# marja-w/gan-des-midi-music-gen

Measured on AMD Instinct MI355X. Metric: GAN training samples/sec (G+D step), higher is better.
Workload: dtype bf16; 1 GPU; SIMNN G/D iteration, synthetic 128x256 spectrogram windows; per_gpu_batch=256, global_batch=256, mode=faithful, parallelism=dp1

## Files before the change

gan_des_midi_music_gen_amd/_lib.py:

```python
import ctypes
import os
import threading

_PKG = os.path.dirname(os.path.abspath(__file__))
_TAG = os.environ.get("GDM_LIB_TAG", "")
LIB_PATH = os.path.join(_PKG, "libgdm_hip" + (f"_{_TAG}" if _TAG else "") + ".so")

F32, BF16 = 0, 1
ACT_NONE, ACT_RELU, ACT_LEAKY, ACT_SIGMOID = 0, 1, 2, 3
CRITERIA = {"bce": 0, "mse": 1, "l1": 2}
PCM_U8, PCM_S16, PCM_S24, PCM_S32, PCM_F32 = range(5)
PCM_BYTES = (1, 2, 3, 4, 4)

_c = ctypes
_P, _I, _L, _F, _Z = _c.c_void_p, _c.c_int, _c.c_int64, _c.c_float, _c.c_size_t

class LinearBnJob(_c.Structure):
    _fields_ = [(n, _P) for n in ("x", "w", "bias", "gamma", "beta", "running_mean", "running_var",
                                  "num_batches_tracked", "y_out", "out", "save_mean", "save_invstd")] + \
               [(n, _I) for n in ("M", "N", "K", "groups", "stat_repeats")]


class DcnnAdam(_c.Structure):
    _fields_ = [("param", _P * 6), ("exp_avg", _P * 6), ("exp_avg_sq", _P * 6), ("hyper", _P), ("done", _P)]


class ConcatJob(_c.Structure):
    _fields_ = [("a", _P), ("b", _P), ("out", _P), ("M", _I), ("Ka", _I), ("Kb", _I)]


SIGNATURES = {
    "gdm_last_error": (_c.c_char_p, []),
    "gdm_version": (_I, []),
    "gdm_arch": (_c.c_char_p, []),
    "gdm_build_flavor": (_I, []),
    "gdm_gemm": (_I, [_P, _I, _L, _L, _P, _I, _L, _L, _P, _I, _L, _L, _I, _I, _I, _P, _P, _I, _F, _I, _I, _P, _Z, _P]),
    "gdm_gemm_plan": (_I, [_P, _I, _L, _L, _P, _I, _L, _L, _P, _I, _L, _L, _I, _I, _I, _P, _I, _I, _P]),
    "gdm_bce_with_logits": (_I, [_P, _F, _I, _F, _P, _P, _I, _I, _P]),
    "gdm_criterion_loss": (_I, [_P, _F, _I, _I, _F, _P, _P, _I, _P]),
    "gdm_adam_step": (_I, [_P, _P, _P, _P, _L, _I, _F, _F, _F, _F, _F, _P]),
    "gdm_adam_step_dev": (_I, [_P, _P, _P, _P, _L, _P, _P]),
    "gdm_adam_step_dev_pc": (_I, [_P, _P, _P, _P, _I, _I, _I, _P, _I, _P, _I, _P]),
    "gdm_stft_frames": (_I, [_P, _I, _L, _L, _I, _I, _I, _P, _P]),
    "gdm_power_spectrum": (_I, [_P, _L, _I, _I, _P, _P]),
    "gdm_power_to_db": (_I, [_P, _I, _I, _I, _F, _F, _P, _P]),
    "gdm_pcm_to_float": (_I, [_P, _I, _I, _I, _L, _L, _L, _P, _P]),
    "gdm_pcm_stft_frames": (_I, [_P, _I, _I, _I, _L, _L, _L, _I, _L, _L, _I, _I, _I, _P, _P]),
    "gdm_bn_workspace_bytes": (_Z, [_I, _I]),
    "gdm_bn_act_fwd": (_I, [_P, _I, _I, _P, _P, _P, _P, _P, _F, _F, _I, _P, _I, _P, _P, _I, _P, _Z, _P]),
    "gdm_bn_act_bwd": (_I, [_P, _P, _I, _P, _I, _I, _P, _P, _P, _I, _P, _P, _P, _P, _Z, _P]),
    "gdm_bn_stats": (_I, [_P, _I, _I, _P, _P, _P, _F, _F, _P, _P, _P, _Z, _P]),
    "gdm_bn_partial_chunks": (_I, [_I]),
    "gdm_bn_partials": (_I, [_P, _I, _I, _P, _P]),
    "gdm_bn_apply": (_I, [_P, _I, _I, _P, _P, _P, _P, _I, _P, _I, _P]),
    "gdm_bn_finalize": (_I, [_P, _I, _I, _I, _F, _F, _P, _P, _P, _P, _P, _P]),
    "gdm_simnn_gen_pack_bytes": (_Z, []),
    "gdm_simnn_gen_pack": (_I, [_P, _I, _P, _P, _P, _P]),
    "gdm_simnn_gen_first": (_I, [_P, _I, _I, _P, _P, _F, _F, _P, _P, _P, _P, _P, _P]),
    "gdm_simnn_gen_convt_chunks": (_I, [_I, _I]),
    "gdm_simnn_gen_convt_bn": (_I, [_I, _P, _P, _P, _P, _P, _I, _P, _P, _P, _P]),
    "gdm_simnn_gen_last": (_I, [_P, _P, _P, _P, _P, _P, _I, _P, _P]),
    "gdm_simnn_gen_eval": (_I, [_P, _I, _I, _P, _P] + [_P] * 12 + [_F, _P, _P, _P, _P, _P, _P]),
    "gdm_bias_act_fwd": (_I, [_P, _P, _I, _I, _I, _F, _P, _I, _P]),
    "gdm_act_bwd": (_I, [_P, _P, _I, _L, _I, _F, _P, _P]),
    "gdm_colsum": (_I, [_P, _I, _I, _I, _P, _P, _Z, _P]),
    "gdm_cast": (_I, [_P, _I, _P, _I, _L, _P]),
    "gdm_nonfinite_count": (_I, [_P, _I, _L, _P, _P]),
    "gdm_simnn_conv1_fwd": (_I, [_P, _P, _P, _I, _I, _I, _P, _P, _I, _P]),
    "gdm_simnn_conv1_fwd_pair": (_I, [_P, _P, _I, _P, _P, _I, _I, _I, _P, _P, _I, _P]),
    "gdm_simnn_conv2_pack_bytes": (_Z, [_I]),
    "gdm_simnn_conv2_pack": (_I, [_P, _I, _P, _P]),
    "gdm_simnn_conv2_fwd": (_I, [_P, _P, _P, _I, _I, _I, _P, _P, _I, _P]),
    "gdm_simnn_conv2_bwd_fused_workspace_bytes": (_Z, [_I, _I, _I]),
    "gdm_simnn_conv2_bwd_fused": (_I, [_P, _P, _P, _I, _I, _I, _P, _P, _P, _I, _I, _I, _P, _I, _P, _Z, _P]),
    "gdm_simnn_conv2_bwd_fused_finish": (_I, [_I, _I, _I, _P, _P, _P, _Z, _P]),
    "gdm_simnn_conv2_bwd_data": (_I, [_P, _P, _P, _I, _I, _I, _P, _I, _P]),
    "gdm_simnn_conv2_bwd_weight_workspace_bytes": (_Z, [_I, _I, _I]),
    "gdm_simnn_conv2_bwd_weight": (_I, [_P, _P, _P, _I, _I, _I, _P, _P, _I, _P, _Z, _P]),
    "gdm_simnn_conv1_bwd_weight_workspace_bytes": (_Z, [_I, _I, _I]),
    "gdm_simnn_conv1_bwd_weight": (_I, [_P, _P, _P, _I, _I, _I, _P, _P, _I, _I, _P, _Z, _P]),
    "gdm_simnn_conv1_bwd_data": (_I, [_P, _P, _P, _I, _I, _I, _P, _I, _P]),
    "gdm_simnn_adam_step": (_I, [_P, _P, _P, _P, _I, _I, _I, _P, _P, _P, _P, _P, _I, _P, _P, _I, _P, _P, _P]),
    "gdm_simnn_head_workspace_bytes": (_Z, [_I]),
    "gdm_simnn_head": (_I, [_P, _P, _P, _I, _I, _F, _F, _P, _P, _I, _P, _I, _P, _P, _P, _P, _Z, _P]),
    "gdm_linear_bn_act_max_rows": (_I, []),
    "gdm_linear_bn_act_fwd_multi": (_I, [_P, _I, _F, _F, _I, _I, _P]),
    "gdm_concat_cols_multi": (_I, [_P, _I, _P]),
    "gdm_linear_bn_act_fwd": (_I, [_P, _P, _P, _P, _P, _P, _P, _P, _F, _F, _I, _I, _I, _I, _I, _P, _P, _P, _P, _I, _I,
                                   _P]),
    "gdm_dcnn_fused_supported": (_I, [_I]),
    "gdm_dcnn_pack_bytes": (_Z, [_I]),
    "gdm_dcnn_pack": (_I, [_P, _P, _P, _P, _P, _P, _I, _P, _P]),
    "gdm_dcnn_fused_workspace_bytes": (_Z, [_I, _I, _I]),
    "gdm_dcnn_fused": (_I, [_P, _I, _P, _P, _I, _I, _F, _F, _P, _P, _P, _I, _I, _P, _P, _P, _P, _P, _P, _P, _Z, _P]),
    "gdm_dcnn_fused_adam": (_I, [_P, _I, _P, _P, _I, _I, _F, _F, _P, _P, _P, _I, _P, _P, _P, _P, _P, _P, _P, _P, _Z, _P]),
    "gdm_dcnn_fused_crit": (_I, [_P, _I, _P, _P, _I, _I, _F, _F, _P, _P, _P, _I, _I, _P, _P, _P, _P, _P, _P, _I, _P, _Z,
                                 _P]),
    "gdm_dcnn_fused_adam_crit": (_I, [_P, _I, _P, _P, _I, _I, _F, _F, _P, _P, _P, _I, _P, _P, _P, _P, _P, _P, _P, _I, _P,
                                      _Z, _P]),
    "gdm_im2col": (_I, [_P, _I, _I, _I, _I, _I, _I, _I, _I, _I, _I, _I, _I, _P, _I, _P]),
    "gdm_col2im": (_I, [_P, _I, _I, _I, _I, _I, _I, _I, _I, _I, _I, _I, _P, _I, _I, _P]),
    "gdm_permute_pc": (_I, [_P, _I, _I, _I, _I, _P, _I, _P]),
    "gdm_des_scan": (_I, [_P, _L, _I, _I, _I, _F, _I, _I, _P, _P, _P, _P, _P, _P, _P]),
    "gdm_des_routing": (_I, [_P, _L, _I, _I, _I, _P, _P, _P, _P]),
    "gdm_des_run": (_I, [_P, _I, _P, _P, _P, _L, _L, _L, _P, _P, _P, _P, _P, _L, _P, _P]),
    "gdm_piano_roll_raster": (_I, [_P, _P, _P, _I, _I, _P, _P, _P]),
    "gdm_piano_roll_windows": (_I, [_P, _P, _P, _P, _P, _I, _I, _P, _P, _P]),
    "gdm_des_log_to_roll": (_I, [_P, _P, _P, _P, _P, _L, _P, _I, _P, _P, _I, _P, _I, _I, _I, _I, _P, _I, _P, _I, _P, _P,
                                 _P]),
    "gdm_maxpool2_fwd": (_I, [_P, _I, _I, _I, _I, _I, _P, _P, _P]),
    "gdm_maxpool2_bwd": (_I, [_P, _I, _P, _I, _I, _I, _I, _P, _P]),
}

_lock = threading.Lock()
_lib = None


class GdmError(RuntimeError):
    pass


def load():
    global _lib
    if _lib is not None:
        return _lib
    with _lock:
        if _lib is None:
            if not os.path.exists(LIB_PATH):
                raise GdmError(
                    f"{LIB_PATH} is missing: build it with `python -m gan_des_midi_music_gen_amd.build` "
                    "(hipcc --offload-arch=gfx950). There is no CPU or eager-PyTorch fallback for this path.")
            import torch
            lib = ctypes.CDLL(LIB_PATH)
            for name, (res, args) in SIGNATURES.items():
                fn = getattr(lib, name)
                fn.restype, fn.argtypes = res, args
            _lib = lib
    return _lib


def check(rc, what):
    if rc != 0:
        msg = load().gdm_last_error().decode(errors="replace")
        raise GdmError(f"{what} failed (rc={rc}): {msg}")
```

gan_des_midi_music_gen_amd/ops.py:

```python
import contextlib
import ctypes
import threading

import torch

from . import _lib
from ._lib import ACT_LEAKY, ACT_NONE, ACT_RELU, ACT_SIGMOID, BF16, CRITERIA, F32, GdmError, check
from ._lib import PCM_BYTES, PCM_F32, PCM_S16, PCM_S24, PCM_S32, PCM_U8

_TORCH_DT = {F32: torch.float32, BF16: torch.bfloat16}


def torch_dtype(dt):
    return _TORCH_DT[dt]


def gdm_dtype(t):
    if t.dtype == torch.float32:
        return F32
    if t.dtype == torch.bfloat16:
        return BF16
    raise GdmError(f"unsupported tensor dtype {t.dtype} (fp32 or bf16 only)")


# ... 486 lines not shown
        assert dw.numel() == 64 and db.numel() == 16 and dw.is_contiguous() and db.is_contiguous()
    else:
        dw = torch.empty((16, 1, 2, 2), dtype=torch.float32, device=x0.device)
        db = torch.empty(16, dtype=torch.float32, device=x0.device)
    dp1 = torch.empty((b, h1, w1, 16), dtype=dp2.dtype, device=dp2.device) if want_dp1 else None
    lib = _lib.load()
    nb = lib.gdm_simnn_conv2_bwd_fused_workspace_bytes(b, h1, w1)
    ws = workspace(nb, x0.device)
    _call("gdm_simnn_conv2_bwd_fused", _p(dp2), _p(code2), _p(pack), b, h1, w1, _p(code1), _p(x0), _p(x1), bsplit, h,
          wd, _p(dp1), gdm_dtype(dp2), _p(ws), nb, _stream())
    _call("gdm_simnn_conv2_bwd_fused_finish", b, h1, w1, _p(dw), _p(db), _p(ws), nb, _stream())
    return dw, db, dp1


def simnn_conv2_bwd_weight(dp2, code2, p1, out=None):
    _need_gpu(dp2, code2, p1)
    assert dp2.is_contiguous() and code2.is_contiguous() and p1.is_contiguous() and dp2.dtype == p1.dtype
    b, h1, w1, _ = p1.shape
    if out is not None:
        dw, db = out
        assert dw.numel() == 4608 and db.numel() == 32 and dw.is_contiguous() and db.is_contiguous()
    else:
        dw = torch.empty((32, 16, 3, 3), dtype=torch.float32, device=p1.device)
        db = torch.empty(32, dtype=torch.float32, device=p1.device)
    lib = _lib.load()
    nb = lib.gdm_simnn_conv2_bwd_weight_workspace_bytes(b, h1, w1)
    ws = workspace(nb, p1.device)
    _call("gdm_simnn_conv2_bwd_weight", _p(dp2), _p(code2), _p(p1), b, h1, w1, _p(dw), _p(db), gdm_dtype(p1), _p(ws),
                                         nb, _stream())
    return dw, db


def simnn_conv1_bwd_weight(dp1, code1, x, out=None, accumulate=False):
    _need_gpu(dp1, code1, x)
    assert dp1.is_contiguous() and code1.is_contiguous() and x.is_contiguous()
    b, h, wd = x.shape
    assert dp1.shape[0] == b and code1.shape == (b, (h + 1) // 2, simnn_code1_width((wd + 1) // 2))
    if out is not None:
        dw, db = out
        assert dw.numel() == 64 and db.numel() == 16 and dw.is_contiguous() and db.is_contiguous()
    else:
        assert not accumulate
        dw = torch.empty((16, 1, 2, 2), dtype=torch.float32, device=x.device)
        db = torch.empty(16, dtype=torch.float32, device=x.device)
    lib = _lib.load()
    nb = lib.gdm_simnn_conv1_bwd_weight_workspace_bytes(b, h, wd)
    ws = workspace(nb, x.device)
    _call("gdm_simnn_conv1_bwd_weight", _p(dp1), _p(code1), _p(x), b, h, wd, _p(dw), _p(db), gdm_dtype(dp1),
                                         1 if accumulate else 0, _p(ws), nb, _stream())
    return dw, db


def simnn_conv1_bwd_data(dp1, code1, w, h, wd):
    _need_gpu(dp1, code1, w)
    assert dp1.is_contiguous() and code1.is_contiguous() and w.is_contiguous() and w.numel() == 64
    b = dp1.shape[0]
    assert dp1.shape == (b, (h + 1) // 2, (wd + 1) // 2, 16)
    assert code1.shape == (b, (h + 1) // 2, simnn_code1_width((wd + 1) // 2))
    dx = torch.empty((b, h, wd), dtype=torch.float32, device=dp1.device)
    _call("gdm_simnn_conv1_bwd_data", _p(dp1), _p(code1), _p(w), b, h, wd, _p(dx), gdm_dtype(dp1), _stream())
    return dx


def simnn_head(h1, w2, b2, n0, y0, y1, *, loss_out, accumulate_loss=False, want_grad=True, grad_out=None, dh_dtype=F32):
    _need_gpu(h1, w2, b2, loss_out)
    assert h1.dim() == 2 and h1.shape[1] == 128 and h1.is_contiguous() and h1.dtype == torch.float32
    n = h1.shape[0]
    prob = torch.empty(n, dtype=torch.float32, device=h1.device)
    dh1 = dw2 = db2 = db1 = None
    if want_grad:
        dh1 = torch.empty(h1.shape, dtype=_TORCH_DT[dh_dtype], device=h1.device)
        if grad_out is not None:
            dw2, db2, db1 = grad_out
            assert dw2.numel() == 128 and db2.numel() == 1 and db1.numel() == 128
        else:
            dw2 = torch.empty((1, 128), dtype=torch.float32, device=h1.device)
            db2 = torch.empty(1, dtype=torch.float32, device=h1.device)
            db1 = torch.empty(128, dtype=torch.float32, device=h1.device)
    nb = _lib.load().gdm_simnn_head_workspace_bytes(n)
    ws = workspace(nb, h1.device)
    _call("gdm_simnn_head", _p(h1), _p(w2), _p(b2), n, n0, float(y0), float(y1), _p(prob), _p(loss_out),
          1 if accumulate_loss else 0, _p(dh1), int(dh_dtype), _p(dw2), _p(db2), _p(db1), _p(ws), nb, _stream())
    return prob, dh1, ((dw2, db2, db1) if want_grad else None)


def linear_bn_act_max_rows():
    return _lib.load().gdm_linear_bn_act_max_rows()


def linear_bn_act_fwd(x, w, bias, gamma, beta, running_mean, running_var, nbt, *, act, training=True, momentum=0.1,
                      eps=1e-5, save_y=False, groups=1, stat_repeats=1):
    _need_gpu(x, w, bias, gamma, beta, running_mean, running_var, nbt)
    assert x.dim() == 2 and w.dim() == 2 and x.shape[1] == w.shape[1] and x.is_contiguous() and w.is_contiguous()
    assert x.dtype == torch.float32 and w.dtype == torch.float32
    rows, k = x.shape
    assert rows % groups == 0
    m = rows // groups
    n = w.shape[0]
    out = torch.empty((rows, n), dtype=torch.float32, device=x.device)
    y = torch.empty((rows, n), dtype=torch.float32, device=x.device) if save_y else None
    shape = (n,) if groups == 1 else (groups, n)
    mean = torch.empty(shape, dtype=torch.float32, device=x.device)
    invstd = torch.empty(shape, dtype=torch.float32, device=x.device)
    _call("gdm_linear_bn_act_fwd", _p(x), _p(w), _p(bias), _p(gamma), _p(beta), _p(running_mean), _p(running_var),
          _p(nbt), float(momentum), float(eps), act, 1 if training else 0, m, n, k, _p(y), _p(out), _p(mean),
          _p(invstd), int(groups), int(stat_repeats), _stream())
    return out, y, mean, invstd


def linear_bn_act_fwd_multi(jobs, *, act, training=True, momentum=0.1, eps=1e-5):
    assert 1 <= len(jobs) <= 2
    arr = (_lib.LinearBnJob * len(jobs))()
    res = []
    for i, j in enumerate(jobs):
        x, w = j["x"], j["w"]
        _need_gpu(x, w, j["bias"], j["gamma"], j["beta"], j["running_mean"], j["running_var"], j["nbt"])
        assert x.dim() == 2 and w.dim() == 2 and x.shape[1] == w.shape[1] and x.is_contiguous() and w.is_contiguous()
        assert x.dtype == torch.float32 and w.dtype == torch.float32
        groups, reps = int(j.get("groups", 1)), int(j.get("stat_repeats", 1))
        rows, k = x.shape
        assert rows % groups == 0
        n = w.shape[0]
        out = torch.empty((rows, n), dtype=torch.float32, device=x.device)
        shape = (n,) if groups == 1 else (groups, n)
        mean = torch.empty(shape, dtype=torch.float32, device=x.device)
        invstd = torch.empty(shape, dtype=torch.float32, device=x.device)
        a = arr[i]
        a.x, a.w, a.bias, a.gamma, a.beta = _p(x), _p(w), _p(j["bias"]), _p(j["gamma"]), _p(j["beta"])
        a.running_mean, a.running_var, a.num_batches_tracked = _p(j["running_mean"]), _p(j["running_var"]), _p(j["nbt"])
        a.y_out, a.out, a.save_mean, a.save_invstd = None, _p(out), _p(mean), _p(invstd)
        a.M, a.N, a.K, a.groups, a.stat_repeats = rows // groups, n, k, groups, reps
        res.append((out, mean, invstd))
    _call("gdm_linear_bn_act_fwd_multi", ctypes.cast(arr, ctypes.c_void_p), len(jobs), float(momentum), float(eps), act,
          1 if training else 0, _stream())
    return res


def concat_cols_multi(pairs, outs=None):
    assert 1 <= len(pairs) <= 4 and (outs is None or len(outs) == len(pairs))
    arr = (_lib.ConcatJob * len(pairs))()
    res = []
    for i, (a, b) in enumerate(pairs):
        _need_gpu(a, b)
        assert a.dim() == 2 and b.dim() == 2 and a.shape[0] == b.shape[0] and a.is_contiguous() and b.is_contiguous()
        assert a.dtype == torch.float32 and b.dtype == torch.float32
        shape = (a.shape[0], a.shape[1] + b.shape[1])
        out = outs[i] if outs is not None else torch.empty(shape, dtype=torch.float32, device=a.device)
        assert tuple(out.shape) == shape and out.is_contiguous() and out.dtype == torch.float32
        q = arr[i]
        q.a, q.b, q.out, q.M, q.Ka, q.Kb = _p(a), _p(b), _p(out), a.shape[0], a.shape[1], b.shape[1]
        res.append(out)
    _call("gdm_concat_cols_multi", ctypes.cast(arr, ctypes.c_void_p), len(pairs), _stream())
    return res


def dcnn_fused_supported(t):
    return bool(_lib.load().gdm_dcnn_fused_supported(int(t)))


def dcnn_pack(w1, b1, w2, b2, wfc, bfc, t, out=None):
    _need_gpu(w1, b1, w2, b2, wfc, bfc, out)
    for a in (w1, b1, w2, b2, wfc, bfc):
        assert a.dtype == torch.float32 and a.is_contiguous()
    nbytes = _lib.load().gdm_dcnn_pack_bytes(int(t))
    pack = out if out is not None else torch.empty(nbytes, dtype=torch.uint8, device=w1.device)
    assert pack.numel() == nbytes
# ... 317 lines not shown
```

gan_des_midi_music_gen_amd/train.py:

```python
import torch

from . import dp
from . import functional as Fn
from . import ops


class FlatBuffers:

    ALIGN = 64

    def __init__(self, params, extra=0, local=0):
        params = [p for p in params]
        assert params, "no parameters"
        dev = params[0].device
        self.params = params
        self.numel = sum(p.numel() for p in params)
        big = max(range(len(params)), key=lambda i: params[i].numel())
        order = [i for i in range(len(params)) if i != big] + [big]
        n_small = self.numel - params[big].numel()
        assert extra % 4 == 0 and 0 <= local <= extra
        self.n_small = (n_small + self.ALIGN - 1) // self.ALIGN * self.ALIGN
        self.n_pad = self.n_small - n_small
        self.n_extra = extra
        self.n_local = local
# ... 128 lines not shown
            torch.cuda.current_stream().wait_event(self._gen_event)

    def _reduce_big_async(self):
        self._pending = dp.allreduce_async_(self.d.bucket_big(), self.pg)

    def _reduce(self):
        pending = self._pending
        if pending is None:
            red = self.d.bucket_reduced()
            dp.allreduce_bucket_(red, red.numel(), self.pg)
        else:
            dp.allreduce_bucket_(self.d.bucket_head(), self.d.bucket_head().numel(), self.pg)
            pending.wait()
            self._pending = None

    def _adam(self):
        self.d.adam(self.lr, self.betas, self.eps, grad_scale=1.0 / self.world)

    def _reduce_and_step(self):
        self._reduce()
        self._adam()

    def _sync_hyper(self):
        self.d.sync_hyper(self.lr, self.betas, self.eps, 1.0 / self.world)

    @torch.no_grad()
    def load_discriminator_state(self, params=None, exp_avg=None, exp_avg_sq=None, step=None):
        d = self.d
        for src, flat in ((params, d.flat), (exp_avg, d.exp_avg), (exp_avg_sq, d.exp_avg_sq)):
            if src is None:
                continue
            assert len(src) == len(d.views)
            for v, s_ in zip(d.views, src):
                off = (v.data_ptr() - d.flat.data_ptr()) // 4
                flat[off:off + v.numel()].copy_(s_.detach().reshape(-1).to(flat.device, torch.float32))
        if step is not None:
            d.step_count = int(step)
            if d._hyper is not None:
                d._hyper.view(torch.int32)[0:1].copy_(torch.tensor([int(step)], dtype=torch.int32))
                if d.derived_record is not None:
                    d.derived_record.zero_()
        if params is not None:
            self._refresh_operands()

    def _count_nonfinite(self, tensors):
        if self._nf is None:
            self._nf = torch.zeros(1, dtype=torch.int32, device=self.d.flat.device)
        ops.nonfinite_count(tensors, self._nf)
        return self._nf

    def _watch(self, *tensors):
        if torch.is_anomaly_enabled():
            self._count_nonfinite([t for t in tensors if isinstance(t, torch.Tensor)])

    def check_finite(self, *tensors):
        nf = self._count_nonfinite([self.loss_g, self.loss_d, self.d.flat, self.d.exp_avg, self.d.exp_avg_sq, *tensors])
        n = int(nf.item())
        nf.zero_()
        if n:
            raise ops.NonFiniteError(f"{type(self).__name__}: {n} non-finite value(s) in inputs, losses, discriminator "
                                     f"parameters or optimizer state after iteration {self.iterations}")

    def _anomaly_check(self):
        if torch.is_anomaly_enabled() and not torch.cuda.is_current_stream_capturing():
            self.check_finite()

    def disc_loss_value(self):
        return self.loss_d.item() / self.world

    def gen_loss_value(self):
        return self.loss_g.item()

    def gen_loss_global(self):
        if self.world == 1:
            return self.loss_g.item()
        t = self.loss_g.clone()
        dp.allreduce_bucket_(t, 1, self.pg)
        return t.item() / self.world


class SimnnTrainer(_TrainerBase):

    def __init__(self, gen, disc, lr=0.00002, betas=(0.5, 0.999), eps=1e-8, compute_dtype=None,
                 elide_dead_backward=False, process_group=None, overlap=True, one_launch_optimizer=True):
        self.gen, self.disc = gen, disc
        self.one_launch_optimizer = one_launch_optimizer
        self._init_common([disc.conv1.weight, disc.conv1.bias, disc.conv2.weight, disc.conv2.bias, disc.fc1.weight,
                           disc.fc1.bias, disc.fc2.weight, disc.fc2.bias], lr, betas, eps, compute_dtype,
                          elide_dead_backward, process_group)
        self._last_generated = None
        self._prepared = None
        self.overlap = overlap
        self._tm_cache = {}
        self._side = None
        self._pending_fake = None
        self._fake_buf = None
        self._pieces = None
        self._piece_streams = None

    @property
    def last_generated(self):
        self._join_generators()
        return self._last_generated

    def invalidate_weights(self):
        self._prepared = None

    def _refresh_operands(self):
        if self._prepared is not None:
            Fn.simnn_disc_prepare(self.d.views[2], self.d.views[4], self.dt, out=self._prepared)

    def _operands(self):
        if self._prepared is None:
            self._prepared = Fn.simnn_disc_prepare(self.d.views[2], self.d.views[4], self.dt)
        return self._prepared

    def _adam(self):
        wf1 = self.d.views[4]
        n, k = wf1.shape
        d = self.d
        if not self.one_launch_optimizer:
            d.adam(self.lr, self.betas, self.eps, grad_scale=1.0 / self.world, big_pc=(n, 32, k // 32, self._prepared[1]))
            ops.simnn_conv2_pack(d.views[2], self.dt, out=self._prepared[0])
            return
        if self._adam_done is None:
            self._adam_done = d.derived_record = torch.zeros(ops.SIMNN_ADAM_RECORD_INTS, dtype=torch.int32,
                                                             device=d.flat.device)
        hyper = d.hyper_record(self.lr, self.betas, self.eps, 1.0 / self.world)
        ns = d.n_small
        ops.simnn_adam_step(d.flat[ns:], d.grad[ns:], d.exp_avg[ns:], d.exp_avg_sq[ns:], n, 32, k // 32, self._prepared[1],
                            d.flat[:ns], d.grad[:ns], d.exp_avg[:ns], d.exp_avg_sq[:ns], d.views[2], self._prepared[0],
                            hyper, self._adam_done)

    def _gen_state(self):
        g = self.gen
        ws = [g.conv1.weight.detach(), g.conv2.weight.detach(), g.conv3.weight.detach(), g.conv4.weight.detach()]
        bns = [(bn.weight.detach(), bn.bias.detach(), bn.running_mean, bn.running_var, bn.num_batches_tracked)
               for bn in (g.batch_norm1, g.batch_norm2, g.batch_norm3)]
        return ws, bns

    def _streams(self, dev, fork=True):
        if not (self.overlap and fork):
            return None
        if self._side is None:
            self._side = [torch.cuda.Stream(dev) for _ in range(3)]
        return self._side

    def _gen_forward(self, noise, keep):
        ws, bns = self._gen_state()
        self._last_generated, gsaved = Fn.simnn_gen_forward(noise, ws, bns, self.gen.training, self.dt,
                                                            cache=self._tm_cache, need_backward=False)
        keep.append(gsaved)
        return self._last_generated

    def _conv1_pair(self, real, fake):
        w1, b1 = self.d.views[:2]
        b, h, w = real.shape
        h1, w1s = (h + 1) // 2, (w + 1) // 2
        p1 = torch.empty((2 * b, h1, w1s, 16), dtype=ops.torch_dtype(self.dt), device=real.device)
        code1 = torch.empty((2 * b, h1, ops.simnn_code1_width(w1s)), dtype=torch.int64, device=real.device)
        ops.simnn_conv1_fwd(real, w1, b1, self.dt, out=(p1[:b], code1[:b]))
        ops.simnn_conv1_fwd(fake, w1, b1, self.dt, out=(p1[b:], code1[b:]))
        return p1, code1

    def _features_head(self, x, trunk, n0, y0, y1, loss_out, grad_out=None, want_grad=True):
        w1, b1, _w2, b2, _wf1, bf1, wf2, bf2 = self.d.views
        pack, wf1p = self._operands()
        hid, saved = Fn.simnn_disc_features(x, w1, b1, pack, b2, wf1p, bf1, self.dt, trunk_out=trunk)
        prob, dh, _ = ops.simnn_head(hid, wf2, bf2, n0, y0, y1, loss_out=loss_out, want_grad=want_grad,
                                     grad_out=grad_out, dh_dtype=self.dt)
        return saved, dh, (hid, prob)

    def _disc_features_head(self, trunk):
        gv = self.d.grad_views
        return self._features_head(None, trunk, trunk[0].shape[0] // 2, 0.9, 0.1, self.loss_d,
                                   grad_out=(gv[6], gv[7], gv[5]))

    def _fc1_dw(self, saved, dh, outs):
        n, k = self._prepared[1].shape
        ops.gemm(dh.t(), saved[3], compute=self.dt, out=outs[4].view(n, k))

    def _backward_rest(self, saved, dh, outs, x_pair, keep):
        _x, p1, code1, _flat, code2 = saved[:5]
        pack, wf1p = self._prepared
        dflat = ops.gemm(dh, wf1p, compute=self.dt, out_dtype=self.dt)
        dp2 = dflat.view(p1.shape[0], p1.shape[1] // 2, p1.shape[2] // 2, 32)
        keep.append(dflat)
        ops.simnn_conv2_bwd_weight(dp2, code2, p1, out=(outs[2], outs[3]))
        ops.simnn_conv2_bwd_fused(dp2, code2, pack, code1, x_pair[0], x_pair[1], out=(outs[0], outs[1]))

    def _d_backward(self, saved, dh, outs, x_pair, keep, fork=True):
        main = torch.cuda.current_stream()
        side = self._streams(saved[1].device, fork)
        if side:
            side[1].wait_stream(main)
        with torch.cuda.stream(side[1] if side else main):
            self._fc1_dw(saved, dh, outs)
            if self.world > 1 and outs is self.d.grad_views:
                self._reduce_big_async()
        self._backward_rest(saved, dh, outs, x_pair, keep)
        if side:
            main.wait_stream(side[1])

    def _generator_half(self, fake, keep, fork=False):
        saved, dh, head = self._features_head(fake, None, fake.shape[0], 1.0, 1.0, self.loss_g,
                                              want_grad=not self.elide)
        if not self.elide:
            self._d_backward(saved, dh, self._scratch(), (fake, None), keep, fork=fork)
        keep.append((saved, dh, head))

    def _gen_forward_beside(self, noise, keep, side):
        main = torch.cuda.current_stream()
        if side:
            side[0].wait_stream(main)
        with torch.cuda.stream(side[0] if side else main):
            return self._gen_forward(noise, keep)

    @torch.no_grad()
    def step(self, real, noise, fake):
        if self._pending_fake is not None:
            self.flush()
        real = Fn._f32c(real)
        self._watch(real, noise, fake)
        main = torch.cuda.current_stream()
        side = self._streams(real.device)
        keep = []
        bridge = callable(fake)
        if bridge:
            generated = self._gen_forward_beside(noise, keep, side)
            if side:
                main.wait_stream(side[0])
            fake = fake(generated)
        fake = Fn._f32c(fake.to(real.device))
        assert fake.shape == real.shape, (fake.shape, real.shape)
        self._operands()
        trunk = self._conv1_pair(real, fake)
        if not bridge:
            self._gen_forward_beside(noise, keep, side)
        saved, dh, head = self._disc_features_head(trunk)
        self._d_backward(saved, dh, self.d.grad_views, (real, fake), keep)
        self._reduce_and_step()
        self._generator_half(fake, keep, fork=True)
        if side:
            main.wait_stream(side[0])
        self.iterations += 1
        del keep, saved, dh, head
        self._anomaly_check()
        return self.loss_d, self.loss_g

    @torch.no_grad()
    def step_pipelined(self, real, noise, fake, with_generator=True):
        if callable(fake):
            raise ops.GdmError("step_pipelined needs a tensor for the fake batch (the bridge is host code)")
        real = Fn._f32c(real)
        fake = Fn._f32c(fake.to(real.device))
        assert fake.shape == real.shape, (fake.shape, real.shape)
        main = torch.cuda.current_stream()
        side = self._streams(real.device)
        keep = []
        pending = self._pending_fake
        self._operands()
        self._scratch()
        trunk = self._conv1_pair(real, fake)
        if with_generator:
            self._gen_forward_beside(noise, keep, side)
        if side:
            side[2].wait_stream(main)
        with torch.cuda.stream(side[2] if side else main):
# ... 415 lines not shown
```

include/gdm.h:

```cpp
#ifndef GDM_H
#define GDM_H
#include <stddef.h>
#include <stdint.h>

#ifdef __cplusplus
extern "C" {
#endif

enum { GDM_F32 = 0, GDM_BF16 = 1 };
enum { GDM_ACT_NONE = 0, GDM_ACT_RELU = 1, GDM_ACT_LEAKY = 2, GDM_ACT_SIGMOID = 3 };
enum { GDM_OK = 0, GDM_EINVAL = -1, GDM_ELAUNCH = -2, GDM_EWORKSPACE = -3 };
enum { GDM_CRIT_BCE_LOGITS = 0, GDM_CRIT_MSE = 1, GDM_CRIT_L1 = 2 };

const char* gdm_last_error(void);
int gdm_version(void);
const char* gdm_arch(void);
int gdm_build_flavor(void);

int gdm_gemm(const void* A, int a_dtype, int64_t sam, int64_t sak,
             const void* B, int b_dtype, int64_t sbk, int64_t sbn,
             void* C, int c_dtype, int64_t scm, int64_t scn,
             int M, int N, int K,
             const float* bias_n, const float* bias_m, int act, float slope,
             int compute_dtype, int split_k, void* workspace, size_t workspace_bytes, void* stream);
// ... 21 lines not shown
int gdm_adam_step_dev_pc(float* p, const float* g_pc, float* m, float* v, int N, int C, int P, void* shadow_pc,
                         int shadow_dtype, float* hyper, int advance_step, void* stream);

size_t gdm_bn_workspace_bytes(int rows, int channels);
int gdm_bn_act_fwd(const float* y, int rows, int channels, const float* gamma, const float* beta,
                   float* running_mean, float* running_var, int64_t* num_batches_tracked, float momentum, float eps,
                   int act, void* out, int out_dtype, float* save_mean, float* save_invstd, int training,
                   void* workspace, size_t workspace_bytes, void* stream);
int gdm_bn_act_bwd(const void* dout, const void* out, int out_dtype, const float* y, int rows, int channels,
                   const float* gamma, const float* save_mean, const float* save_invstd, int act, float* dy,
                   float* dgamma, float* dbeta, void* workspace, size_t workspace_bytes, void* stream);
int gdm_bn_stats(const float* y, int rows, int channels, float* running_mean, float* running_var,
                 int64_t* num_batches_tracked, float momentum, float eps, float* save_mean, float* save_invstd,
                 void* workspace, size_t workspace_bytes, void* stream);
int gdm_bn_partial_chunks(int rows);
int gdm_bn_partials(const float* y, int rows, int channels, float* partials, void* stream);
int gdm_bn_apply(const float* y, int rows, int channels, const float* gamma, const float* beta, const float* mean,
                 const float* invstd, int act, void* out, int out_dtype, void* stream);
int gdm_bn_finalize(const float* ws, int chunks, int rows, int channels, float momentum, float eps, float* running_mean,
                    float* running_var, int64_t* num_batches_tracked, float* save_mean, float* save_invstd, void* stream);

size_t gdm_simnn_gen_pack_bytes(void);
int gdm_simnn_gen_pack(const float* w1, int noise_dim, const float* w2, const float* w3, void* pack, void* stream);
int gdm_simnn_gen_first(const float* noise, int B, int noise_dim, const void* pack, float* y1, float momentum, float eps,
                        float* running_mean, float* running_var, int64_t* num_batches_tracked, float* save_mean,
                        float* save_invstd, void* stream);
int gdm_simnn_gen_convt_chunks(int layer, int B);
int gdm_simnn_gen_convt_bn(int layer, const float* yin, const float* mean, const float* invstd, const float* gamma,
                           const float* beta, int B, const void* pack, float* yout, float* ws_partials, void* stream);
int gdm_simnn_gen_last(const float* yin, const float* mean, const float* invstd, const float* gamma, const float* beta,
                       const float* w4, int B, float* out, void* stream);
int gdm_simnn_gen_eval(const float* noise, int B, int noise_dim, const void* pack, const float* w4,
                       const float* gamma1, const float* beta1, const float* rmean1, const float* rvar1,
                       const float* gamma2, const float* beta2, const float* rmean2, const float* rvar2,
                       const float* gamma3, const float* beta3, const float* rmean3, const float* rvar3,
                       float eps, float* out, float* tap_y1, float* tap_y2, float* tap_y3, float* tap_invstd,
                       void* stream);


int gdm_bias_act_fwd(const float* x, const float* bias, int rows, int cols, int act, float slope, void* out,
                     int out_dtype, void* stream);
int gdm_act_bwd(const void* dout, const void* out, int dtype, int64_t n, int act, float slope, void* dx, void* stream);
int gdm_colsum(const void* x, int dtype, int rows, int cols, float* out, void* workspace, size_t workspace_bytes,
               void* stream);
int gdm_cast(const void* src, int src_dtype, void* dst, int dst_dtype, int64_t n, void* stream);
int gdm_nonfinite_count(const void* x, int dtype, int64_t n, int* counter, void* stream);

int gdm_simnn_conv1_fwd(const float* x, const float* w, const float* bias, int B, int H, int W, void* p1,
                        uint64_t* code1, int dtype, void* stream);
int gdm_simnn_conv1_fwd_pair(const float* x0, const float* x1, int bsplit, const float* w, const float* bias, int B,
                             int H, int W, void* p1, uint64_t* code1, int dtype, void* stream);
size_t gdm_simnn_conv2_pack_bytes(int dtype);
int gdm_simnn_conv2_pack(const float* w, int dtype, void* pack, void* stream);
int gdm_simnn_conv2_fwd(const void* p1, const void* pack, const float* bias, int B, int H1, int W1, void* p2,
                        uint8_t* code2, int dtype, void* stream);
int gdm_simnn_conv2_bwd_data(const void* dp2, const uint8_t* code2, const void* pack, int B, int H1, int W1, void* dp1,
                             int dtype, void* stream);
size_t gdm_simnn_conv2_bwd_fused_workspace_bytes(int B, int H1, int W1);
int gdm_simnn_conv2_bwd_fused(const void* dp2, const uint8_t* code2, const void* pack, int B, int H1, int W1,
                              const uint64_t* code1, const float* x0, const float* x1, int bsplit, int H, int W,
                              void* dp1_or_null, int dtype, void* workspace, size_t workspace_bytes, void* stream);
int gdm_simnn_conv2_bwd_fused_finish(int B, int H1, int W1, float* dw1, float* db1, void* workspace,
                                     size_t workspace_bytes, void* stream);
size_t gdm_simnn_conv2_bwd_weight_workspace_bytes(int B, int H1, int W1);
int gdm_simnn_conv2_bwd_weight(const void* dp2, const uint8_t* code2, const void* p1, int B, int H1, int W1,
                               float* dw, float* db, int dtype, void* workspace, size_t workspace_bytes, void* stream);
size_t gdm_simnn_conv1_bwd_weight_workspace_bytes(int B, int H, int W);
int gdm_simnn_conv1_bwd_weight(const void* dp1, const uint64_t* code1, const float* x, int B, int H, int W,
                               float* dw, float* db, int dtype, int accumulate, void* workspace, size_t workspace_bytes,
                               void* stream);
int gdm_simnn_conv1_bwd_data(const void* dp1, const uint64_t* code1, const float* w, int B, int H, int W, float* dx,
                             int dtype, void* stream);

#define GDM_SIMNN_ADAM_RECORD_INTS 1056
int gdm_simnn_adam_step(float* p_big, const float* g_big_pc, float* m_big, float* v_big, int N, int C, int P,
                        void* shadow_pc, float* p_small, const float* g_small, float* m_small, float* v_small,
                        int n_small, const float* conv2_weight, void* pack, int dtype, float* hyper, int* done,
                        void* stream);

size_t gdm_simnn_head_workspace_bytes(int n);
int gdm_simnn_head(const float* h1, const float* w2, const float* b2, int n, int n0, float y0, float y1, float* prob,
                   float* loss, int accumulate_loss, void* dh1, int dh1_dtype ,
                   float* dw2, float* db2, float* db1, void* workspace, size_t workspace_bytes, void* stream);

typedef struct gdm_linear_bn_job {
  const float *x, *w, *bias, *gamma, *beta;
  float *running_mean, *running_var;
  int64_t* num_batches_tracked;
  float *y_out, *out, *save_mean, *save_invstd;
  int M, N, K, groups, stat_repeats;
} gdm_linear_bn_job;
int gdm_linear_bn_act_max_rows(void);
int gdm_linear_bn_act_fwd_multi(const gdm_linear_bn_job* jobs, int n_jobs, float momentum, float eps, int act,
                                int training, void* stream);
typedef struct gdm_concat_job {
  const float *a, *b;
  float* out;
  int M, Ka, Kb;
} gdm_concat_job;
int gdm_concat_cols_multi(const gdm_concat_job* jobs, int n_jobs, void* stream);
int gdm_linear_bn_act_fwd(const float* x, const float* w, const float* bias, const float* gamma, const float* beta,
                          float* running_mean, float* running_var, int64_t* num_batches_tracked, float momentum,
                          float eps, int act, int training, int M, int N, int K, float* y_out, float* out,
                          float* save_mean, float* save_invstd, int groups, int stat_repeats, void* stream);
int gdm_dcnn_fused_supported(int T);
size_t gdm_dcnn_pack_bytes(int T);
int gdm_dcnn_pack(const float* w1, const float* b1, const float* w2, const float* b2, const float* wfc,
                  const float* bfc, int T, void* pack, void* stream);
size_t gdm_dcnn_fused_workspace_bytes(int B, int T, int want_grad);
int gdm_dcnn_fused(const float* xa, int bsplit, const float* p0, const float* p1, int B, int T, float ya, float yb,
                   const void* pack, float* logits, float* loss, int accumulate_loss, int want_grad, float* dw1,
                   float* db1, float* dw2, float* db2, float* dwfc, float* dbfc, void* workspace,
                   size_t workspace_bytes, void* stream);
typedef struct gdm_dcnn_adam {
  float* param[6];
  float* exp_avg[6];
  float* exp_avg_sq[6];
  float* hyper;
  int* done;
} gdm_dcnn_adam;
int gdm_dcnn_fused_adam(const float* xa, int bsplit, const float* p0, const float* p1, int B, int T, float ya, float yb,
                        void* pack, float* logits, float* loss, int accumulate_loss, float* dw1, float* db1, float* dw2,
                        float* db2, float* dwfc, float* dbfc, const gdm_dcnn_adam* opt, void* workspace,
                        size_t workspace_bytes, void* stream);
int gdm_dcnn_fused_crit(const float* xa, int bsplit, const float* p0, const float* p1, int B, int T, float ya, float yb,
                        const void* pack, float* logits, float* loss, int accumulate_loss, int want_grad, float* dw1,
                        float* db1, float* dw2, float* db2, float* dwfc, float* dbfc, int criterion, void* workspace,
                        size_t workspace_bytes, void* stream);
int gdm_dcnn_fused_adam_crit(const float* xa, int bsplit, const float* p0, const float* p1, int B, int T, float ya,
                             float yb, void* pack, float* logits, float* loss, int accumulate_loss, float* dw1,
                             float* db1, float* dw2, float* db2, float* dwfc, float* dbfc, const gdm_dcnn_adam* opt,
                             int criterion, void* workspace, size_t workspace_bytes, void* stream);

typedef struct gdm_des_event {
  double value;
  int64_t event_id;
  int32_t node;
  int32_t kind;
} gdm_des_event;
int gdm_des_run(const double* adj, int dim, const double* loc, const double* scale, const int32_t* queue_cap, int64_t seed,
                int64_t number_of_customers, int64_t max_events, uint32_t* mt_key, int* mt_pos, int* has_gauss,
                double* cached_gauss, gdm_des_event* out, int64_t out_capacity, int64_t* n_out, int* stop_reason);

int gdm_im2col(const void* src, int src_dtype, int src_planar, int B, int H, int W, int C, int KH, int KW,
               int stride, int pad, int OH, int OW, void* cols, int cols_dtype, void* stream);
int gdm_col2im(const void* cols, int cols_dtype, int B, int H, int W, int C, int KH, int KW, int stride, int pad,
               int OH, int OW, void* dst, int dst_dtype, int dst_planar, void* stream);

int gdm_permute_pc(const void* src, int src_dtype, int B, int P, int C, void* dst, int dst_dtype, void* stream);

int gdm_maxpool2_fwd(const void* src, int dtype, int B, int H, int W, int C, void* dst, uint8_t* idx_or_null,
                     void* stream);
int gdm_maxpool2_bwd(const void* dout, int dtype, const uint8_t* idx, int B, int H, int W, int C, void* dx,
                     void* stream);

int gdm_des_scan(const float* g, int64_t sample_stride, int B, int S, int dim, float threshold, int note_mod,
                 int norm_aux, uint8_t* thr_mask_or_null, int32_t* instruments, int32_t* note_levels,
                 uint64_t* zero_mask, float* aux_or_null, int32_t* flags, void* stream);
int gdm_des_routing(const float* g, int64_t sample_stride, int B, int S, int dim, const uint8_t* src_mask,
                    const int32_t* residue_col, double* out, void* stream);

int gdm_piano_roll_raster(const int32_t* row_ptr, const int32_t* ev_step, const int32_t* ev_vel, int n_files, int W,
                          float* roll, float* dur, void* stream);

int gdm_piano_roll_windows(const int32_t* row_ptr, const int32_t* ev_step, const int32_t* ev_vel,
                           const int32_t* win_file, const int32_t* win_s0, int n_windows, int L, float* roll,
// ... 42 lines not shown
```

Measured before the change: 424,900 samples/s.

## Add streaming fc1 data-gradient kernel keeping dh in registers across column tiles

Adds a dedicated HIP kernel for the fc1 backward data GEMM (K=128). Each workgroup keeps its dh row tile in registers and walks many output column tiles, double-buffering weight panels in LDS and writing bf16 through an LDS transpose. It replaces the generic gemm call when shapes allow, aiming to avoid repeated A loads and K-loop overhead of the general kernel. It adds a specialized code path and falls back to the generic gemm otherwise.

New measurement: 426,100 samples/s (median of 6 runs). Within noise of the previous version (+0.3%).

```diff
diff --git a/gan_des_midi_music_gen_amd/_lib.py b/gan_des_midi_music_gen_amd/_lib.py
--- a/gan_des_midi_music_gen_amd/_lib.py
+++ b/gan_des_midi_music_gen_amd/_lib.py
@@ -83,6 +83,8 @@
     "gdm_simnn_adam_step": (_I, [_P, _P, _P, _P, _I, _I, _I, _P, _P, _P, _P, _P, _I, _P, _P, _I, _P, _P, _P]),
     "gdm_simnn_head_workspace_bytes": (_Z, [_I]),
     "gdm_simnn_head": (_I, [_P, _P, _P, _I, _I, _F, _F, _P, _P, _I, _P, _I, _P, _P, _P, _P, _Z, _P]),
+    "gdm_simnn_fc1_dx_workgroups": (_I, [_I, _I]),
+    "gdm_simnn_fc1_dx": (_I, [_P, _I, _P, _I, _I, _P, _I, _P]),
     "gdm_linear_bn_act_max_rows": (_I, []),
     "gdm_linear_bn_act_fwd_multi": (_I, [_P, _I, _F, _F, _I, _I, _P]),
     "gdm_concat_cols_multi": (_I, [_P, _I, _P]),
diff --git a/gan_des_midi_music_gen_amd/csrc/simnn_fc1_bwd.hip b/gan_des_midi_music_gen_amd/csrc/simnn_fc1_bwd.hip
--- /dev/null
+++ b/gan_des_midi_music_gen_amd/csrc/simnn_fc1_bwd.hip
@@ -0,0 +1,153 @@
+#include "gemm_bf16_kernel.h"
+
+namespace {
+
+constexpr int FC1_HIDDEN = 128;
+constexpr int DX_WORKGROUPS = 512;
+constexpr int DX_IMG = FC1_HIDDEN * BN;
+constexpr size_t DX_LDS_BYTES = 2 * DX_IMG * sizeof(__bf16) + 4 * 16 * 64 * sizeof(float);
+
+inline int dx_walkers(int M, int N) {
+  const int MT = M / BM, NTl = N / BN;
+  int c = (DX_WORKGROUPS / MT) & ~7;
+  if (c < 8) c = 8;
+  const int need = (NTl + 7) & ~7;
+  return c < need ? c : need;
+}
+
+template <typename TA>
+__global__ __launch_bounds__(NT, 2) void fc1_dx_kernel(const TA* __restrict__ dh, const __bf16* __restrict__ wpc,
+                                                       __bf16* __restrict__ out, int M, int N, int walkers) {
+  extern __shared__ __attribute__((aligned(16))) __bf16 dx_smem[];
+  const int t = threadIdx.x, l = t & 63, w = t >> 6, wm = w >> 1, wn = w & 1;
+  const int lr = l & 15, lg = l >> 4;
+  const int MT = M / BM, NTl = N / BN;
+  const int id = blockIdx.x;
+  const int grp = id / (8 * MT), within = id % (8 * MT);
+  const int c = grp * 8 + (within & 7), mt = within >> 3;
+  if (c >= NTl) return;
+  const int m0 = mt * BM;
+  const rsrc_t ra = make_rsrc(dh, (uint32_t)((int64_t)M * FC1_HIDDEN * (int64_t)sizeof(TA)));
+  const rsrc_t rb = make_rsrc(wpc, (uint32_t)((int64_t)FC1_HIDDEN * N * (int64_t)sizeof(__bf16)));
+  const rsrc_t rc = make_rsrc(out, (uint32_t)((int64_t)M * N * (int64_t)sizeof(__bf16)));
+
+  Lane<__bf16, FC1_HIDDEN> lb;
+  lane_init<__bf16, FC1_HIDDEN, false>(lb, N, N, 0);
+  Stage<__bf16, FC1_HIDDEN> sb;
+  auto panel_load = [&](int nt) {
+    const bool ok = nt < NTl;
+    const uint32_t col = ok ? (uint32_t)(nt * BN * (int)sizeof(__bf16)) : 0u;
+#pragma unroll
+    for (int i = 0; i < Stage<__bf16, FC1_HIDDEN>::N; ++i)
+      sb.v[i] = __builtin_bit_cast(f32x4, __builtin_amdgcn_raw_buffer_load_b128(rb, ok ? lb.off[i] : BUF_OOB, col, 0));
+  };
+
+  bf16x8 a[4][4];
+#pragma unroll
+  for (int i = 0; i < 4; ++i)
+#pragma unroll
+    for (int kk = 0; kk < 4; ++kk) {
+      const uint32_t e = (uint32_t)((m0 + wm * 64 + 16 * i + lr) * FC1_HIDDEN + 32 * kk + 8 * lg);
+      if constexpr (sizeof(TA) == 2) {
+        a[i][kk] = __builtin_bit_cast(bf16x8, buf_load16(ra, e * 2u));
+      } else {
+        const f32x4 lo = buf_load16(ra, e * 4u), hi = buf_load16(ra, e * 4u + 16u);
+#pragma unroll
+        for (int r = 0; r < 4; ++r) {
+          a[i][kk][r] = (__bf16)lo[r];
+          a[i][kk][4 + r] = (__bf16)hi[r];
+        }
+      }
+    }
+
+  float* scr = (float*)(dx_smem + 2 * DX_IMG) + w * (16 * 64);
+  const int prow = l >> 3, c8 = l & 7;
+  const uint32_t out_lane = (uint32_t)(((m0 + wm * 64 + prow) * (int64_t)N + wn * 64 + 8 * c8) * (int64_t)sizeof(__bf16));
+  const uint32_t out_row8 = (uint32_t)(8 * (int64_t)N * (int64_t)sizeof(__bf16));
+
+  panel_load(c);
+  stage_store<__bf16, FC1_HIDDEN>(sb, lb, dx_smem);
+  panel_load(c + walkers);
+  int buf = 0;
+  for (int nt = c; nt < NTl; nt += walkers, buf ^= 1) {
+    const __bf16* Bs = dx_smem + buf * DX_IMG;
+    __syncthreads();
+
+    f32x4 acc[4][4];
+#pragma unroll
+    for (int i = 0; i < 4; ++i)
+#pragma unroll
+      for (int j = 0; j < 4; ++j) acc[i][j] = (f32x4){0.f, 0.f, 0.f, 0.f};
+#pragma unroll
+    for (int kk = 0; kk < 4; ++kk) {
+      bf16x8 b[4];
+#pragma unroll
+      for (int j = 0; j < 4; ++j) b[j] = frag_read<FC1_HIDDEN, false>(Bs, wn * 64 + 16 * j, kk, lr, lg);
+#pragma unroll
+      for (int i = 0; i < 4; ++i)
+#pragma unroll
+        for (int j = 0; j < 4; ++j) acc[i][j] = mfma16(b[j], a[i][kk], acc[i][j]);
+    }
+
+    const uint32_t col = (uint32_t)(nt * BN * (int)sizeof(__bf16));
+#pragma unroll
+    for (int i = 0; i < 4; ++i) {
+      wave_lds_sync();
+#pragma unroll
+      for (int j = 0; j < 4; ++j) *(f32x4*)&scr[lr * 64 + 4 * ((4 * j + lg) ^ lr)] = acc[i][j];
+      wave_lds_sync();
+#pragma unroll
+      for (int h = 0; h < 2; ++h) {
+        const int row = 8 * h + prow;
+        const f32x4 v0 = *(const f32x4*)&scr[row * 64 + 4 * ((2 * c8) ^ row)];
+        const f32x4 v1 = *(const f32x4*)&scr[row * 64 + 4 * ((2 * c8 + 1) ^ row)];
+        bf16x8 hv;
+#pragma unroll
+        for (int r = 0; r < 4; ++r) {
+          hv[r] = (__bf16)v0[r];
+          hv[4 + r] = (__bf16)v1[r];
+        }
+        __builtin_amdgcn_raw_buffer_store_b128(__builtin_bit_cast(u32x4, hv), rc,
+                                               out_lane + (uint32_t)(2 * i + h) * out_row8, col, 2);
+      }
+    }
+    stage_store<__bf16, FC1_HIDDEN>(sb, lb, dx_smem + (buf ^ 1) * DX_IMG);
+    panel_load(nt + 2 * walkers);
+  }
+}
+
+inline bool aligned16(const void* p) { return ((uintptr_t)p & 15) == 0; }
+
+}
+
+extern "C" int gdm_simnn_fc1_dx_workgroups(int M, int N) {
+  if (M <= 0 || N <= 0 || M % BM || N % BN) return 0;
+  return dx_walkers(M, N) * (M / BM);
+}
+
+extern "C" int gdm_simnn_fc1_dx(const void* dh, int dh_dtype, const void* w_pc, int M, int N, void* out, int dtype,
+                                void* stream) {
+  GDM_REQUIRE(dtype == GDM_BF16, "gdm_simnn_fc1_dx: bf16 compute only (got dtype %d)", dtype);
+  GDM_REQUIRE(gdm_dtype_ok(dh_dtype), "gdm_simnn_fc1_dx: bad dh dtype %d", dh_dtype);
+  GDM_REQUIRE(M > 0 && N > 0 && M % BM == 0 && N % BN == 0, "gdm_simnn_fc1_dx: M = %d and N = %d must be multiples of 128",
+              M, N);
+  GDM_REQUIRE(dh && w_pc && out && aligned16(dh) && aligned16(w_pc) && aligned16(out),
+              "gdm_simnn_fc1_dx: operands must be 16-byte aligned");
+  const int64_t lim = (int64_t)1 << 31;
+  GDM_REQUIRE((int64_t)M * N * 2 < lim && (int64_t)FC1_HIDDEN * N * 2 < lim &&
+                  (int64_t)M * FC1_HIDDEN * (int64_t)gdm_dtype_size(dh_dtype) < lim,
+              "gdm_simnn_fc1_dx: every tensor must be below 2 GiB (M = %d, N = %d)", M, N);
+  const dim3 grid((unsigned)(dx_walkers(M, N) * (M / BM)));
+  hipStream_t s = (hipStream_t)stream;
+  if (dh_dtype == GDM_BF16) {
+    allow_lds(fc1_dx_kernel<__bf16>, DX_LDS_BYTES);
+    hipLaunchKernelGGL(fc1_dx_kernel<__bf16>, grid, dim3(NT), DX_LDS_BYTES, s, (const __bf16*)dh, (const __bf16*)w_pc,
+                       (__bf16*)out, M, N, dx_walkers(M, N));
+  } else {
+    allow_lds(fc1_dx_kernel<float>, DX_LDS_BYTES);
+    hipLaunchKernelGGL(fc1_dx_kernel<float>, grid, dim3(NT), DX_LDS_BYTES, s, (const float*)dh, (const __bf16*)w_pc,
+                       (__bf16*)out, M, N, dx_walkers(M, N));
+  }
+  GDM_LAUNCH_OK("gdm_simnn_fc1_dx");
+  return GDM_OK;
+}
diff --git a/gan_des_midi_music_gen_amd/ops.py b/gan_des_midi_music_gen_amd/ops.py
--- a/gan_des_midi_music_gen_amd/ops.py
+++ b/gan_des_midi_music_gen_amd/ops.py
@@ -592,6 +592,35 @@
     _call("gdm_simnn_head", _p(h1), _p(w2), _p(b2), n, n0, float(y0), float(y1), _p(prob), _p(loss_out),
           1 if accumulate_loss else 0, _p(dh1), int(dh_dtype), _p(dw2), _p(db2), _p(db1), _p(ws), nb, _stream())
     return prob, dh1, ((dw2, db2, db1) if want_grad else None)
+
+
+def simnn_fc1_dx_ok(dh, w_pc, out, compute):
+    if compute != BF16 or dh.dim() != 2 or w_pc.dim() != 2 or dh.shape[1] != 128 or w_pc.shape[0] != 128:
+        return False
+    m, n = dh.shape[0], w_pc.shape[1]
+    if m == 0 or n == 0 or m % 128 or n % 128 or m * n * 2 >= 1 << 31:
+        return False
+    if dh.dtype not in (torch.float32, torch.bfloat16) or w_pc.dtype != torch.bfloat16:
+        return False
+    if out is not None and (out.shape != (m, n) or out.dtype != torch.bfloat16):
+        return False
+    return all(t is None or (t.is_contiguous() and t.data_ptr() % 16 == 0 and t.numel() * t.element_size() < 1 << 31)
+               for t in (dh, w_pc, out))
+
+
+def simnn_fc1_dx_workgroups(m, n):
+    return _lib.load().gdm_simnn_fc1_dx_workgroups(m, n)
+
+
+def simnn_fc1_dx(dh, w_pc, compute, out=None):
+    if not simnn_fc1_dx_ok(dh, w_pc, out, compute):
+        return None
+    _need_gpu(dh, w_pc, out)
+    m, n = dh.shape[0], w_pc.shape[1]
+    if out is None:
+        out = torch.empty((m, n), dtype=torch.bfloat16, device=dh.device)
+    _call("gdm_simnn_fc1_dx", _p(dh), gdm_dtype(dh), _p(w_pc), m, n, _p(out), compute, _stream())
+    return out
 
 
 def linear_bn_act_max_rows():
diff --git a/gan_des_midi_music_gen_amd/train.py b/gan_des_midi_music_gen_amd/train.py
--- a/gan_des_midi_music_gen_amd/train.py
+++ b/gan_des_midi_music_gen_amd/train.py
@@ -234,9 +234,11 @@
 class SimnnTrainer(_TrainerBase):
 
     def __init__(self, gen, disc, lr=0.00002, betas=(0.5, 0.999), eps=1e-8, compute_dtype=None,
-                 elide_dead_backward=False, process_group=None, overlap=True, one_launch_optimizer=True):
+                 elide_dead_backward=False, process_group=None, overlap=True, one_launch_optimizer=True,
+                 fc1_streaming_backward=True):
         self.gen, self.disc = gen, disc
         self.one_launch_optimizer = one_launch_optimizer
+        self.fc1_streaming_backward = fc1_streaming_backward
         self._init_common([disc.conv1.weight, disc.conv1.bias, disc.conv2.weight, disc.conv2.bias, disc.fc1.weight,
                            disc.fc1.bias, disc.fc2.weight, disc.fc2.bias], lr, betas, eps, compute_dtype,
                           elide_dead_backward, process_group)
@@ -335,7 +337,9 @@
     def _backward_rest(self, saved, dh, outs, x_pair, keep):
         _x, p1, code1, _flat, code2 = saved[:5]
         pack, wf1p = self._prepared
-        dflat = ops.gemm(dh, wf1p, compute=self.dt, out_dtype=self.dt)
+        dflat = ops.simnn_fc1_dx(dh, wf1p, self.dt) if self.fc1_streaming_backward else None
+        if dflat is None:
+            dflat = ops.gemm(dh, wf1p, compute=self.dt, out_dtype=self.dt)
         dp2 = dflat.view(p1.shape[0], p1.shape[1] // 2, p1.shape[2] // 2, 32)
         keep.append(dflat)
         ops.simnn_conv2_bwd_weight(dp2, code2, p1, out=(outs[2], outs[3]))
diff --git a/include/gdm.h b/include/gdm.h
--- a/include/gdm.h
+++ b/include/gdm.h
@@ -127,6 +127,9 @@
 int gdm_simnn_head(const float* h1, const float* w2, const float* b2, int n, int n0, float y0, float y1, float* prob,
                    float* loss, int accumulate_loss, void* dh1, int dh1_dtype ,
                    float* dw2, float* db2, float* db1, void* workspace, size_t workspace_bytes, void* stream);
+
+int gdm_simnn_fc1_dx_workgroups(int M, int N);
+int gdm_simnn_fc1_dx(const void* dh, int dh_dtype, const void* w_pc, int M, int N, void* out, int dtype, void* stream);
 
 typedef struct gdm_linear_bn_job {
   const float *x, *w, *bias, *gamma, *beta;
```
